# TengdaHan/TemporalAlignNet

Hardware: AMD Instinct MI355X
Metric: video-seq/sec (len=64, E6D6) at 1/2/4/8 MI355X; HTM-Align ROC-AUC parity (higher is better)
Workload: dtype bf16; 1 GPU; E6D6 len=64 bf16 stage-1 (init: multi-positive NCE only) train step (fwd+loss+bwd+AdamW), synthetic HTM-370K-shaped features, N~U[4,16] sentences/video; global_batch=128, per_gpu_batch=128, seq_len=64, parallelism=dp1

## Files before the change

### temporalalignnet_amd/csrc/tan_simnce.hip

```cpp
#include <type_traits>

#include "tan_mma.h"

namespace tal {

constexpr float S_TAU = 0.07f;
constexpr int S_TILE = 128 * 64 * 2;
constexpr int S_MAXCOLS = 2048;
constexpr int S_MAXCOLS_RES = 8192;

typedef const void __attribute__((address_space(1)))* sgptr_t;
typedef void __attribute__((address_space(3)))* slptr_t;

struct FamPtrs { void* p[8]; };
struct SimArgs {
    const bf16_t* V;
    const bf16_t* Tt;
    long t_stage_stride;
    const float* tgt;
    const unsigned char* col_invalid;
    const unsigned char* row_leak;
    float *rowsum, *possum_v;
    float *colpart, *pospart;
    const float *colsum, *possum_t;
// ... 11 lines not shown
    float* inv_v;
};

__device__ __forceinline__ void s_stage(const bf16_t* __restrict__ P, long ld, int outer0, int OUT, int k0, char* lds_tile,
                                        int wave, int lane) {
#pragma unroll
    for (int i = 0; i < 4; ++i) {
        const int piece = wave * 4 + i;
        const int row = piece * 8 + (lane >> 3), slot = lane & 7;
        const int chunk = slot ^ ((row >> 1) & 7);
        const int gr = min(outer0 + row, OUT - 1);
        __builtin_amdgcn_global_load_lds((sgptr_t)(P + (long)gr * ld + k0 + chunk * 8), (slptr_t)(lds_tile + piece * 1024), 16, 0, 0);
    }
}
__device__ __forceinline__ bf16x8 s_frag(const char* lds_tile, int o0, int ks, int lane) {
    const int row = o0 + (lane & 31), chunk = (ks >> 3) + (lane >> 5);
    return *reinterpret_cast<const bf16x8*>(lds_tile + row * 128 + (chunk ^ ((row >> 1) & 7)) * 16);
}

struct TileCtx {
    const unsigned char* col_invalid;
    const float* colsum; const float* g_t; bf16_t* dl;
    int R, Mp, s, m0, wm, wn, lane;
    float inv_tau;
    int cinv[2];
};

template <int MODE>
__device__ __forceinline__ void tile_done(const TileCtx& c, f32x16 (&acc)[2][2], float (&rowacc)[2][16], float* colacc, int ct) {
    const int c0 = ct * 128, R = c.R, Mp = c.Mp, lane = c.lane;
#pragma unroll
    for (int j = 0; j < 2; ++j) {
        const int col = c0 + c.wn * 64 + j * 32 + acc_col(lane);
        const bool col_ok = col < Mp;
        const bool col_valid = col_ok && !c.col_invalid[min(col, Mp - 1)];
        float csum = 0.f, bc = 0.f;
        if (MODE == 1) {
            const long idx = (long)c.s * Mp + min(col, Mp - 1);
            const float gt = c.g_t[idx], cs = c.colsum[idx];
            bc = col_ok ? gt / cs * c.inv_tau : 0.f;
        }
#pragma unroll
        for (int i = 0; i < 2; ++i)
#pragma unroll
            for (int r = 0; r < 16; ++r) {
                const int row = c.m0 + c.wm * 64 + i * 32 + acc_row(r, lane);
                float e = __expf((acc[i][j][r] - 1.0f) * c.inv_tau);
                if (!col_ok || row >= R) e = 0.f;
                if (MODE == 0) {
                    if (col_valid) rowacc[i][r] += e;
                    csum += e;
                } else {
                    const float g = e * ((col_valid ? rowacc[i][r] : 0.f) + bc);
                    if (col_ok && row < R) c.dl[((long)c.s * R + row) * Mp + col] = f2bf(g);
                }
            }
        if (MODE == 0 && col_ok) atomicAdd(&colacc[col], csum);
    }
}

template <int MODE>
__global__ __launch_bounds__(256, 2) void simnce_kernel(SimArgs a) {
    __shared__ __attribute__((aligned(1024))) char lds[4 * S_TILE + (MODE == 0 ? S_MAXCOLS * 4 : 0)];
    float* colacc = reinterpret_cast<float*>(lds + 4 * S_TILE);
    const int tid = threadIdx.x, lane = tid & 63;
    const int wave = __builtin_amdgcn_readfirstlane(tid >> 6);
    const int wm = wave >> 1, wn = wave & 1;
    const int npanel = gridDim.x;
    int wg = blockIdx.y * gridDim.x + blockIdx.x;
    {
        const int nwg = gridDim.x * gridDim.y, xcd = wg & 7, q = nwg >> 3, r = nwg & 7;
        wg = (xcd < r ? xcd * (q + 1) : r * (q + 1) + (xcd - r) * q) + (wg >> 3);
    }
    const int s = wg / npanel, panel = wg - s * npanel, m0 = panel * 128;
    const int R = a.R, Mp = a.Mp, Cw = a.C, nS = a.S;
    const bf16_t* V = a.V + (long)s * R * Cw;
    const bf16_t* Tt = a.Tt + (long)s * a.t_stage_stride;
    const int nk = Cw / 64, nct = (Mp + 127) / 128, nsteps = nct * nk;
    const float inv_tau = 1.0f / S_TAU;

    if (MODE == 0) {
        for (int c = tid; c < S_MAXCOLS; c += 256) colacc[c] = 0.f;
    }
    float rowacc[2][16];
#pragma unroll
    for (int i = 0; i < 2; ++i)
#pragma unroll
        for (int r = 0; r < 16; ++r) {
            rowacc[i][r] = 0.f;
            if (MODE == 1) {
                const int row = m0 + wm * 64 + i * 32 + acc_row(r, lane);
                const long idx = (long)s * R + min(row, R - 1);
                const float gv = a.g_v[idx], rs = a.rowsum[idx];
                rowacc[i][r] = row < R ? gv / rs * inv_tau : 0.f;
            }
        }
    TileCtx c;
    c.col_invalid = a.col_invalid; c.colsum = a.colsum; c.g_t = a.g_t; c.dl = a.dl;
    c.R = R; c.Mp = Mp; c.s = s; c.m0 = m0; c.wm = wm; c.wn = wn; c.lane = lane; c.inv_tau = inv_tau;

    f32x16 acc[2][2];
#define SIM_KSTEP(STEP, CUR, NXT)                                                                                          \
    {                                                                                                                      \
        const int step_ = (STEP);                                                                                          \
        const int ct_ = step_ / nk, kt_ = step_ - ct_ * nk;                                                                \
        if (step_ + 1 < nsteps) {                                                                                          \
            const int ct2 = (step_ + 1) / nk, kt2 = (step_ + 1) - ct2 * nk;                                                \
            s_stage(V, Cw, m0, R, kt2 * 64, lds + (NXT) * 2 * S_TILE, wave, lane);                                         \
            s_stage(Tt, Cw, ct2 * 128, Mp, kt2 * 64, lds + (NXT) * 2 * S_TILE + S_TILE, wave, lane);                       \
        }                                                                                                                  \
        if (kt_ == 0) {                                                                                                    \
            _Pragma("unroll") for (int i = 0; i < 2; ++i) _Pragma("unroll") for (int j = 0; j < 2; ++j) acc_zero(acc[i][j]); \
        }                                                                                                                  \
        _Pragma("unroll") for (int ks = 0; ks < 64; ks += 16) {                                                            \
            bf16x8 af[2], bfr[2];                                                                                          \
            _Pragma("unroll") for (int i = 0; i < 2; ++i) af[i] = s_frag(lds + (CUR) * 2 * S_TILE, wm * 64 + i * 32, ks, lane); \
            _Pragma("unroll") for (int j = 0; j < 2; ++j)                                                                  \
                bfr[j] = s_frag(lds + (CUR) * 2 * S_TILE + S_TILE, wn * 64 + j * 32, ks, lane);                            \
            _Pragma("unroll") for (int i = 0; i < 2; ++i) _Pragma("unroll") for (int j = 0; j < 2; ++j)                    \
                acc[i][j] = __builtin_amdgcn_mfma_f32_32x32x16_bf16(af[i], bfr[j], acc[i][j], 0, 0, 0);                    \
        }                                                                                                                  \
        if (kt_ == nk - 1) tile_done<MODE>(c, acc, rowacc, colacc, ct_);                                   \
        asm volatile("s_waitcnt vmcnt(0)" ::: "memory");                                                                   \
        __syncthreads();                                                                                                   \
    }

    s_stage(V, Cw, m0, R, 0, lds, wave, lane);
    s_stage(Tt, Cw, 0, Mp, 0, lds + S_TILE, wave, lane);
    asm volatile("s_waitcnt vmcnt(0)" ::: "memory");
    __syncthreads();
    for (int step = 0; step < nsteps; step += 2) {
        SIM_KSTEP(step, 0, 1)
        if (step + 1 < nsteps) SIM_KSTEP(step + 1, 1, 0)
    }
#undef SIM_KSTEP

    if (MODE == 0) {
#pragma unroll
        for (int i = 0; i < 2; ++i)
#pragma unroll
            for (int r = 0; r < 16; ++r) {
                float v = rowacc[i][r];
#pragma unroll
                for (int o = 16; o > 0; o >>= 1) v += __shfl_xor(v, o, 64);
                const int row = m0 + wm * 64 + i * 32 + acc_row(r, lane);
                if ((lane & 31) == 0 && row < R) unsafeAtomicAdd(a.rowsum + (long)s * R + row, v);
            }
        __syncthreads();
        float* cp = a.colpart + ((long)panel * nS + s) * Mp;
        for (int cc = tid; cc < Mp; cc += 256) cp[cc] = colacc[cc];
    }
}

template <int MODE>
__device__ __forceinline__ void tile_done_res(const TileCtx& c, f32x16 (&acc)[2][2], float (&rowacc)[2][16], float* colrow, int ct) {
    const int c0 = ct * 128, R = c.R, Mp = c.Mp, lane = c.lane;
#pragma unroll
    for (int j = 0; j < 2; ++j) {
        const int col = c0 + c.wn * 64 + j * 32 + acc_col(lane);
        const bool col_ok = col < Mp;
        const bool col_valid = col_ok && !(c.cinv[j] >= 0 ? c.cinv[j] : (int)c.col_invalid[min(col, Mp - 1)]);
        float csum = 0.f, bc = 0.f, e_prev = 0.f;
        unsigned pk[4] = {0u, 0u, 0u, 0u};
        const float k1 = 1.4426950408889634f * c.inv_tau, cmask = col_ok ? 1.0f : 0.0f, vmask = col_valid ? 1.0f : 0.0f;
        const bool rows_full = c.m0 + 128 <= R;
        if (MODE == 1) {
            const long idx = (long)c.s * Mp + min(col, Mp - 1);
            const float gt = c.g_t[idx], cs = c.colsum[idx];
            bc = col_ok ? gt / cs * c.inv_tau : 0.f;
        }
#pragma unroll
        for (int i = 0; i < 2; ++i)
#pragma unroll
            for (int r = 0; r < 16; ++r) {
                const int row = c.m0 + c.wm * 64 + i * 32 + acc_row(r, lane);
                float e = __builtin_amdgcn_exp2f(fmaf(acc[i][j][r], k1, -k1)) * cmask;
                if (!rows_full && row >= R) e = 0.f;
                if (MODE == 0) {
                    rowacc[i][r] = fmaf(e, vmask, rowacc[i][r]);
                    csum += e;
                    if (c.dl) {
                        if (r & 1) pk[(r >> 1) & 3] = f2bf2(e_prev, e);
                        e_prev = e;
                        if ((r & 7) == 7)
                            reinterpret_cast<uint4*>(c.dl)[((i * 2 + j) * 2 + (r >> 3)) * 64 + lane] = make_uint4(pk[0], pk[1], pk[2], pk[3]);
                    }
                } else {
                    const float g = e * ((col_valid ? rowacc[i][r] : 0.f) + bc);
                    if (col_ok && row < R) c.dl[((long)c.s * R + row) * Mp + col] = f2bf(g);
                }
            }
        if (MODE == 0) {
            csum += __shfl_xor(csum, 32, 64);
            if (lane < 32 && col_ok) colrow[col] = csum;
        }
    }
}

template <int J, int END, typename F>
__device__ __forceinline__ void pn_static_for_s(F&& f) {
    if constexpr (J < END) {
        f(std::integral_constant<int, J>{});
        pn_static_for_s<J + 1, END>(f);
    }
}

__global__ __launch_bounds__(256) void simnce_pack_text_kernel(const bf16_t* __restrict__ Tt, long t_stage_stride, char* __restrict__ Tp,
                                                               long tp_stage_stride, int Mp, float* __restrict__ zero, long nzero) {
    const int cb = blockIdx.x, st = blockIdx.y, lane = threadIdx.x & 63, w = threadIdx.x >> 6;
    if (zero)
        for (long i = ((long)blockIdx.y * gridDim.x + blockIdx.x) * 256 + threadIdx.x; i < nzero; i += (long)gridDim.x * gridDim.y * 256) zero[i] = 0.f;
    const bf16_t* src = Tt + (long)st * t_stage_stride + (long)min(cb * 32 + (lane & 31), Mp - 1) * 512 + 8 * (lane >> 5);
    char* dst = Tp + (long)st * tp_stage_stride + (long)cb * 32 * 1024 + lane * 16;
    uint4 v[8];
#pragma unroll
    for (int i = 0; i < 8; ++i) v[i] = *reinterpret_cast<const uint4*>(src + (w * 8 + i) * 16);
#pragma unroll
    for (int i = 0; i < 8; ++i) *reinterpret_cast<uint4*>(dst + (long)(w * 8 + i) * 1024) = v[i];
}

template <int MODE>
__global__ __launch_bounds__(512) void simnce_res_kernel(SimArgs a) {
    __shared__ __attribute__((aligned(1024))) char lds[8 * S_TILE];
    const int tid = threadIdx.x, lane = tid & 63;
    const int wave = __builtin_amdgcn_readfirstlane(tid >> 6);
    const int grp = wave >> 2, gw = wave & 3, wm = gw >> 1, wn = gw & 1;
    const int npanel = a.npanel;
    int wg = blockIdx.x, half = -1;
    if (wg < a.nfull) {
        const int nwg = a.nfull, xcd = wg & 7, q = nwg >> 3, r = nwg & 7;
        wg = (xcd < r ? xcd * (q + 1) : r * (q + 1) + (xcd - r) * q) + (wg >> 3);
    } else {
        half = (wg - a.nfull) & 1;
        wg = a.nfull + ((wg - a.nfull) >> 1);
    }
    const int s = wg / npanel, panel = wg - s * npanel, m0 = panel * 128;
    const int R = a.R, Mp = a.Mp, Cw = a.C, nS = a.S;
    const bf16_t* V = a.V + (long)s * R * Cw;
    const int nct = (Mp + 127) / 128;
    const float inv_tau = 1.0f / S_TAU;

    float rowacc[2][16];
#pragma unroll
    for (int i = 0; i < 2; ++i)
#pragma unroll
        for (int r = 0; r < 16; ++r) {
            rowacc[i][r] = 0.f;
            if (MODE == 1) {
                const int row = m0 + wm * 64 + i * 32 + acc_row(r, lane);
                const long idx = (long)s * R + min(row, R - 1);
                const float gv = a.g_v[idx], rs = a.rowsum[idx];
                rowacc[i][r] = row < R ? gv / rs * inv_tau : 0.f;
            }
        }
    TileCtx c;
    c.col_invalid = a.col_invalid; c.colsum = a.colsum; c.g_t = a.g_t; c.dl = a.dl;
    c.R = R; c.Mp = Mp; c.s = s; c.m0 = m0; c.wm = wm; c.wn = wn; c.lane = lane; c.inv_tau = inv_tau;
    float* colrow = MODE == 0 ? a.colpart + ((long)(2 * panel + wm) * nS + s) * Mp : nullptr;

    f32x16 acc[2][2];
    constexpr int RD = MODE == 0 ? 8 : 4;
    struct BF { bf16x8 f[2]; };
    BF ring[RD];
    const char* Tp = a.Tp + (long)s * a.tp_stage_stride;
    auto load_b = [&](BF& dst, int ct, int ks) __attribute__((always_inline)) {
        const char* pb = Tp + ((long)((ct * 4 + wn * 2) * 32 + ks)) * 1024 + lane * 16;
        dst.f[0] = *reinterpret_cast<const bf16x8*>(pb);
        dst.f[1] = *reinterpret_cast<const bf16x8*>(pb + 32 * 1024);
    };
    const int nall = (nct - grp + 1) / 2;
    const int kbase = half == 1 ? (nall + 1) / 2 : 0;
    const int ngrp = half < 0 ? nall : (half == 0 ? (nall + 1) / 2 : nall / 2);
    const int rot = ngrp > 0 ? (panel * 7 + s * 3) % ngrp : 0;
    if (ngrp > 0) {
        pn_static_for_s<0, RD>([&](auto jc) { constexpr int J = decltype(jc)::value; load_b(ring[J], 2 * (kbase + rot) + grp, J); });
    }
    if (MODE == 0 && a.inv_v) {
        const bf16_t* X = reinterpret_cast<const bf16_t*>(a.xraw.p[s]);
#pragma unroll
        for (int kt = 0; kt < 4; ++kt) {
            char* tile = lds + (grp * 4 + kt) * S_TILE;
#pragma unroll
            for (int i = 0; i < 4; ++i) {
                const int piece = gw * 4 + i;
                const int row = piece * 8 + (lane >> 3), slot = lane & 7;
                const int chunk = slot ^ ((row >> 1) & 7);
                const int gr = min(m0 + row, R - 1);
                const long sr = (long)(gr / a.T) * a.x_grp_rows + a.x_off + gr % a.T;
                __builtin_amdgcn_global_load_lds((sgptr_t)(X + sr * Cw + (grp * 4 + kt) * 64 + chunk * 8), (slptr_t)(tile + piece * 1024), 16, 0, 0);
            }
        }
        asm volatile("s_waitcnt vmcnt(0)" ::: "memory");
        __syncthreads();
        bf16_t* vout = const_cast<bf16_t*>(V);
#pragma unroll 1
        for (int i0 = 0; i0 < 16; i0 += 4) {
            uint4 raw[4];
            char* ap[4];
#pragma unroll
            for (int j = 0; j < 4; ++j) {
                const int row = wave * 16 + i0 + j;
                ap[j] = lds + (lane >> 3) * S_TILE + row * 128 + (((lane & 7) ^ ((row >> 1) & 7)) * 16);
                raw[j] = *reinterpret_cast<const uint4*>(ap[j]);
            }
#pragma unroll
            for (int j = 0; j < 4; ++j) {
                const int row = wave * 16 + i0 + j;
                const unsigned w[4] = {raw[j].x, raw[j].y, raw[j].z, raw[j].w};
                float x[8];
#pragma unroll
                for (int e = 0; e < 4; ++e) { x[2 * e] = __uint_as_float(w[e] << 16); x[2 * e + 1] = __uint_as_float(w[e] & 0xffff0000u); }
                float q = ((x[0] * x[0] + x[1] * x[1]) + (x[2] * x[2] + x[3] * x[3])) + ((x[4] * x[4] + x[5] * x[5]) + (x[6] * x[6] + x[7] * x[7]));
                const float inv = 1.0f / sqrtf(wave_sum(q));
                uint4 y;
                y.x = f2bf2(x[0] * inv, x[1] * inv); y.y = f2bf2(x[2] * inv, x[3] * inv);
                y.z = f2bf2(x[4] * inv, x[5] * inv); y.w = f2bf2(x[6] * inv, x[7] * inv);
                *reinterpret_cast<uint4*>(ap[j]) = y;
                if (m0 + row < R) {
                    *reinterpret_cast<uint4*>(vout + (long)(m0 + row) * Cw + lane * 8) = y;
                    if (lane == 0) a.inv_v[(long)s * R + m0 + row] = inv;
                }
            }
        }
    } else {
#pragma unroll
        for (int kt = 0; kt < 4; ++kt) s_stage(V, Cw, m0, R, (grp * 4 + kt) * 64, lds + (grp * 4 + kt) * S_TILE, gw, lane);
        asm volatile("s_waitcnt vmcnt(0)" ::: "memory");
    }
    __syncthreads();
    bf16x8 afA[2], afB[2];
#pragma unroll
    for (int i = 0; i < 2; ++i) afA[i] = s_frag(lds, wm * 64 + i * 32, 0, lane);
    for (int it = 0; it < ngrp; ++it) {
        const int k_ = it + rot < ngrp ? it + rot : it + rot - ngrp, kn_ = k_ + 1 < ngrp ? k_ + 1 : 0;
        const int ct_ = 2 * (kbase + k_) + grp, ctn_ = 2 * (kbase + kn_) + grp;
        const bool more = it + 1 < ngrp;
#pragma unroll
        for (int i = 0; i < 2; ++i)
#pragma unroll
            for (int j = 0; j < 2; ++j) acc_zero(acc[i][j]);
#pragma unroll
        for (int j = 0; j < 2; ++j) c.cinv[j] = a.col_invalid[min(ct_ * 128 + wn * 64 + j * 32 + (lane & 31), Mp - 1)];
        pn_static_for_s<0, 32>([&](auto jc) {
            constexpr int KS = decltype(jc)::value;
            BF& Bf = ring[KS % RD];
            bf16x8(&af)[2] = (KS & 1) ? afB : afA;
            bf16x8(&an)[2] = (KS & 1) ? afA : afB;
#ifndef TAN_SIM_LAB
#define TAN_SIM_LAB 0
#endif
            if constexpr (!(TAN_SIM_LAB & 2)) {
                constexpr int KN = (KS + 1) & 31;
                const char* vn_ = lds + (KN >> 2) * S_TILE;
#pragma unroll
                for (int i = 0; i < 2; ++i) an[i] = s_frag(vn_, wm * 64 + i * 32, (KN & 3) * 16, lane);
            } else {
#pragma unroll
                for (int i = 0; i < 2; ++i) asm volatile("" : "+v"(an[i]));
            }
#pragma unroll
            for (int i = 0; i < 2; ++i)
#pragma unroll
                for (int j = 0; j < 2; ++j) acc[i][j] = __builtin_amdgcn_mfma_f32_32x32x16_bf16(af[i], Bf.f[j], acc[i][j], 0, 0, 0);
            if constexpr (!(TAN_SIM_LAB & 1)) {
                if constexpr (KS + RD < 32) load_b(Bf, ct_, KS + RD);
                else if (more) load_b(Bf, ctn_, KS + RD - 32);
            } else {
                asm volatile("" : "+v"(Bf.f[0]), "+v"(Bf.f[1]));
            }
            __builtin_amdgcn_sched_barrier(0);
        });
        if (MODE == 0 && a.ekeep && !(TAN_SIM_LAB & 4)) c.dl = a.ekeep + ((((long)s * npanel + panel) * nct + ct_) * 4 + gw) * 4096;
        if constexpr (!(TAN_SIM_LAB & 8)) tile_done_res<MODE>(c, acc, rowacc, colrow, ct_);
        else {
#pragma unroll
            for (int i = 0; i < 2; ++i)
#pragma unroll
                for (int j = 0; j < 2; ++j) asm volatile("" : "+v"(acc[i][j]));
        }
    }

    if (MODE == 0) {
#pragma unroll
        for (int i = 0; i < 2; ++i)
#pragma unroll
            for (int r = 0; r < 16; ++r) {
                float v = rowacc[i][r];
#pragma unroll
                for (int o = 16; o > 0; o >>= 1) v += __shfl_xor(v, o, 64);
                const int row = m0 + wm * 64 + i * 32 + acc_row(r, lane);
                if ((lane & 31) == 0 && row < R) unsafeAtomicAdd(a.rowsum + (long)s * R + row, v);
            }
    }
    if (MODE == 1 && a.diag) {
        asm volatile("s_waitcnt vmcnt(0)" ::: "memory");
        __builtin_amdgcn_fence(__ATOMIC_RELEASE, "workgroup");
        __syncthreads();
        __builtin_amdgcn_fence(__ATOMIC_ACQUIRE, "workgroup");
        const int T = a.T, N = a.N;
        const int nrow = min(128, R - m0);
        for (int i = tid; i < nrow * N; i += 512) {
            const int lr = i / N, k = i - lr * N, row = m0 + lr;
            const int b = row / T, t = row - b * T;
            const int m = a.colmap ? a.colmap[b * N + k] : b * N + k;
            if (m < 0) continue;
            bf16_t* out = a.dl + ((long)s * R + row) * Mp + m;
            if (a.row_leak && a.row_leak[row]) { *out = 0; continue; }
            if (a.tgt[((long)b * T + t) * N + k] == 0.f) continue;
            const long ri = (long)s * R + row, ci = (long)s * Mp + m;
            const float e = __expf((a.diag[(((long)s * a.B + b) * T + t) * N + k] - 1.0f) * inv_tau);
            const float pv = a.possum_v[ri], pt = a.possum_t[ci];
            float corr = 0.f;
            if (!a.col_invalid[m] && pv > 0.f) corr += a.g_v[ri] / pv;
            if (pt > 0.f) corr += a.g_t[ci] / pt;
            *out = f2bf(bf2f(*out) - e * corr * inv_tau);
        }
    }
}

__global__ __launch_bounds__(256) void simnce_dl_kept_kernel(SimArgs a, int npanel, int nct) {
    constexpr int LD = 136;
    __shared__ __attribute__((aligned(16))) bf16_t tile[128 * LD];
    __shared__ float rf[128], cf[128];
    __shared__ unsigned char cv[128];
    __shared__ int crange[2];
    const int tid = threadIdx.x, s = blockIdx.y;
    const int panel = blockIdx.x / nct, ct = blockIdx.x - panel * nct;
    const int R = a.R, Mp = a.Mp, T = a.T, N = a.N, m0 = panel * 128, c0 = ct * 128;
    const float inv_tau = 1.0f / S_TAU;
    if (tid == 0) { crange[0] = 0x7fffffff; crange[1] = -1; }
    __syncthreads();
    if (a.diag) {
        const int b_lo = m0 / T, b_hi = min(m0 + 127, R - 1) / T;
        for (int p = b_lo * N + tid; p < (b_hi + 1) * N; p += 256) {
            const int m = a.colmap ? a.colmap[p] : p;
            if (m >= 0) { atomicMin(&crange[0], m); atomicMax(&crange[1], m); }
        }
    }
    if (tid < 128) {
        const long ri = (long)s * R + min(m0 + tid, R - 1);
        rf[tid] = a.g_v[ri] / a.rowsum[ri] * inv_tau;
    } else {
        const int c = tid - 128, col = min(c0 + c, Mp - 1);
        const long ci = (long)s * Mp + col;
        cf[c] = a.g_t[ci] / a.colsum[ci] * inv_tau;
        cv[c] = !a.col_invalid[col];
    }
    __syncthreads();
    const uint4* E = reinterpret_cast<const uint4*>(a.ekeep) + (((long)s * npanel + panel) * nct + ct) * 2048;
    uint4 ev[8];
#pragma unroll
    for (int n = 0; n < 8; ++n) ev[n] = E[tid + 256 * n];
#pragma unroll
    for (int n = 0; n < 8; ++n) {
        const int v = tid + 256 * n;
        const int gw = v >> 9, ij = (v >> 7) & 3, q = (v >> 6) & 1, ln = v & 63;
        const int col = (gw & 1) * 64 + (ij & 1) * 32 + (ln & 31);
        const unsigned w[4] = {ev[n].x, ev[n].y, ev[n].z, ev[n].w};
        const float c = cf[col];
        const bool ok = cv[col];
#pragma unroll
        for (int j = 0; j < 4; ++j) {
            const int row = (gw >> 1) * 64 + (ij >> 1) * 32 + acc_row(8 * q + 2 * j, ln);
            tile[row * LD + col] = f2bf(__uint_as_float(w[j] << 16) * ((ok ? rf[row] : 0.f) + c));
            tile[(row + 1) * LD + col] = f2bf(__uint_as_float(w[j] & 0xffff0000u) * ((ok ? rf[row + 1] : 0.f) + c));
        }
    }
    __syncthreads();
    if (a.diag && crange[0] <= c0 + 127 && crange[1] >= c0) {
        const int nrow = min(128, R - m0);
        for (int i = tid; i < nrow * N; i += 256) {
            const int lr = i / N, k = i - lr * N, row = m0 + lr;
            const int b = row / T, t = row - b * T;
            const int m = a.colmap ? a.colmap[b * N + k] : b * N + k;
            if (m < c0 || m >= c0 + 128 || m >= Mp) continue;
            bf16_t* out = tile + lr * LD + (m - c0);
            if (a.row_leak && a.row_leak[row]) { *out = 0; continue; }
            if (a.tgt[((long)b * T + t) * N + k] == 0.f) continue;
            const long ri = (long)s * R + row, ci = (long)s * Mp + m;
            const float e = __expf((a.diag[(((long)s * a.B + b) * T + t) * N + k] - 1.0f) * inv_tau);
            const float pv = a.possum_v[ri], pt = a.possum_t[ci];
            float corr = 0.f;
            if (!a.col_invalid[m] && pv > 0.f) corr += a.g_v[ri] / pv;
            if (pt > 0.f) corr += a.g_t[ci] / pt;
            *out = f2bf(bf2f(*out) - e * corr * inv_tau);
        }
        __syncthreads();
    }
    const bool vec = (Mp & 7) == 0;
    for (int q = tid; q < 128 * 16; q += 256) {
        const int lr = q >> 4, cc = (q & 15) * 8, row = m0 + lr, col = c0 + cc;
        if (row >= R || col >= Mp) continue;
        bf16_t* dst = a.dl + ((long)s * R + row) * Mp + col;
        if (vec) *reinterpret_cast<uint4*>(dst) = *reinterpret_cast<const uint4*>(tile + lr * LD + cc);
        else for (int j = 0; j < 8 && col + j < Mp; ++j) dst[j] = tile[lr * LD + cc + j];
    }
}

__global__ __launch_bounds__(256) void simnce_corr_kernel(const float* __restrict__ diag, const float* __restrict__ tgt,
                                                          const unsigned char* __restrict__ col_invalid, const unsigned char* __restrict__ row_leak,
                                                          const float* __restrict__ possum_v, const float* __restrict__ possum_t,
                                                          const float* __restrict__ g_v, const float* __restrict__ g_t, float* __restrict__ corr,
                                                          int B, int T, int N, const int* __restrict__ colmap, int Mp,
                                                          float* __restrict__ zero = nullptr, long nzero = 0) {
    const int b = blockIdx.x, s = blockIdx.y;
    const int R = B * T;
    const float inv_tau = 1.0f / S_TAU;
    const float* blk = diag + ((long)s * B + b) * T * N;
    const float* tg = tgt + (long)b * T * N;
    float* out = corr + ((long)s * B + b) * T * N;
    if (zero)
        for (long i = ((long)blockIdx.y * gridDim.x + blockIdx.x) * 256 + threadIdx.x; i < nzero; i += (long)gridDim.x * gridDim.y * 256) zero[i] = 0.f;
    constexpr int U = 4;
    for (int i0 = threadIdx.x; i0 < T * N; i0 += 256 * U) {
        int cc[U]; long r[U], c[U]; bool in[U], leak[U];
        float tgv[U], bl[U], pv[U], gv[U], pt[U], gt[U]; unsigned char inval[U];
#pragma unroll
        for (int j = 0; j < U; ++j) {
            const int i = min(i0 + j * 256, T * N - 1);
            const int t = i / N, k = i - t * N;
            const int m = colmap ? colmap[b * N + k] : b * N + k;
            in[j] = m >= 0 && m < Mp;
            cc[j] = min(max(m, 0), Mp - 1);
            r[j] = (long)s * R + b * T + t;
            c[j] = (long)s * Mp + cc[j];
            leak[j] = row_leak && row_leak[b * T + t];
            tgv[j] = tg[i]; bl[j] = blk[i]; inval[j] = col_invalid[cc[j]];
            pv[j] = possum_v[r[j]]; gv[j] = g_v[r[j]]; pt[j] = possum_t[c[j]]; gt[j] = g_t[c[j]];
        }
#pragma unroll
        for (int j = 0; j < U; ++j) {
            if (i0 + j * 256 >= T * N) continue;
            float v = 0.f;
            if (in[j]) {
                if (leak[j]) v = INFINITY;
                else if (tgv[j] != 0.f) {
                    const float e = __expf((bl[j] - 1.0f) * inv_tau);
                    float cr = 0.f;
                    if (!inval[j] && pv[j] > 0.f) cr += gv[j] / pv[j];
                    if (pt[j] > 0.f) cr += gt[j] / pt[j];
                    v = e * cr * inv_tau;
                }
            }
            out[i0 + j * 256] = v;
        }
    }
}
// ... 358 lines not shown
                              const unsigned char* __restrict__ col_invalid, int ncols, const float* __restrict__ colsum,
                              const float* __restrict__ possum_t, float* __restrict__ t_terms, long SM, float log_rows) {
    const float log_cols = (long)blockIdx.x * blockDim.x < SR ? block_log_count_zero(col_invalid, ncols) : 0.f;
    const long i = (long)blockIdx.x * blockDim.x + threadIdx.x;
    if (i >= SR + SM) return;
    const bool rows = i < SR;
    const long k = rows ? i : i - SR;
    const float all = rows ? rowsum[k] : colsum[k], pos = rows ? possum_v[k] : possum_t[k], lc = rows ? log_cols : log_rows;
    const float shift = 1.0f / S_TAU;
    const float den = logf(all) + shift;
    const float num = pos > 0.f ? logf(pos) + shift : -6e4f + lc;
    (rows ? v_terms : t_terms)[k] = den - num;
}

}

using namespace tal;

extern "C" int tan_simnce_max_cols(void) {
    SimArgs a{};
    a.C = 512;
    return res_enabled(a) ? S_MAXCOLS_RES : S_MAXCOLS;
}

static long simnce_corr_floats(int S, int B, int T, int N) { return (long)S * B * T * N + 128 * 32 + 8; }

extern "C" long tan_simnce_ws_floats(int S, int B, int T, int N) {
    const long R = (long)B * T, Mp = (long)B * N;
    return 2 * (long)cdiv(R, 128) * S * Mp + (long)S * B * T * N + (long)S * cdiv(Mp, 128) * 128 * 512 / 2 + 4 + simnce_corr_floats(S, B, T, N);
}
static float* simnce_corr_ptr(float* ws, int S, int B, int T, int N) {
    const long R = (long)B * T, Mp = (long)B * N;
    float* p = ws + 2 * (long)cdiv(R, 128) * S * Mp + (long)S * B * T * N + (long)S * cdiv(Mp, 128) * 128 * 512 / 2 + 4;
    return (float*)(((uintptr_t)p + 15) & ~(uintptr_t)15);
}
static int simnce_corr_launch(const SimArgs& a, const float* diag, float* corr, hipStream_t st) {
    hipLaunchKernelGGL(simnce_corr_kernel, dim3(a.B, a.S), dim3(256), 0, st, diag, a.tgt, a.col_invalid, a.row_leak, (const float*)a.possum_v,
                       a.possum_t, a.g_v, a.g_t, corr, a.B, a.T, a.N, a.colmap, a.Mp);
    hipError_t e = hipGetLastError();
    return e == hipSuccess ? 0 : (int)e;
}

static int simnce_common(SimArgs& a, int S, int B, int T, int N, int C) {
    a.S = S; a.B = B; a.T = T; a.N = N; a.C = C; a.R = B * T; a.Mp = B * N;
    if (S <= 0 || B <= 0 || T <= 0 || N <= 0 || C <= 0 || C % 64 != 0) return TAN_ERR_BAD_ARG;
    if (((uintptr_t)a.V % 16) || ((uintptr_t)a.Tt % 16)) return TAN_ERR_BAD_ARG;
    return 0;
}

__global__ __launch_bounds__(256) void simnce_blocks_kernel(const bf16_t* __restrict__ V, const bf16_t* __restrict__ tn_blocks,
                                                            long tb_stage_stride, float* __restrict__ diag, int B, int T, int N, long R) {
    constexpr int C = 512;
    const int b = blockIdx.x, s = blockIdx.y, lane = threadIdx.x & 63, wave = threadIdx.x >> 6;
    const int t0 = (blockIdx.z * 4 + wave) * 32;
    if (t0 >= T) return;
    const int hi8 = 8 * (lane >> 5);
    const bf16_t* arow = V + ((long)s * R + (long)b * T + min(t0 + (lane & 31), T - 1)) * C + hi8;
    float* out = diag + ((long)s * B + b) * T * N;
    for (int n0 = 0; n0 < N; n0 += 32) {
        const bf16_t* brow = tn_blocks + (long)s * tb_stage_stride + ((long)b * N + min(n0 + (lane & 31), N - 1)) * C + hi8;
        f32x16 acc;
        acc_zero(acc);
#pragma unroll 8
        for (int ks = 0; ks < C; ks += 16) {
            const bf16x8 fa = *reinterpret_cast<const bf16x8*>(arow + ks);
            const bf16x8 fb = *reinterpret_cast<const bf16x8*>(brow + ks);
            acc = __builtin_amdgcn_mfma_f32_32x32x16_bf16(fa, fb, acc, 0, 0, 0);
        }
        const int n = n0 + acc_col(lane);
#pragma unroll
        for (int r = 0; r < 16; ++r) {
            const int t = t0 + acc_row(r, lane);
            if (t < T && n < N) out[t * N + n] = acc[r];
        }
    }
}

static int simnce_diag_blocks(const SimArgs& a, const bf16_t* tn_blocks, long tb_stage_stride, float* diag, hipStream_t st) {
    if (a.C == 512 && (((uintptr_t)a.V | (uintptr_t)tn_blocks) % 16) == 0 && tb_stage_stride % 8 == 0) {
        hipLaunchKernelGGL(simnce_blocks_kernel, dim3(a.B, a.S, cdiv(a.T, 128)), dim3(256), 0, st, a.V, tn_blocks, tb_stage_stride, diag,
                           a.B, a.T, a.N, (long)a.R);
        hipError_t e = hipGetLastError();
        return e == hipSuccess ? 0 : (int)e;
    }
    const bool one_launch = tb_stage_stride == (long)a.B * a.N * a.C;
    for (int s = 0; s < (one_launch ? 1 : a.S); ++s) {
        tan_gemm_desc d{};
        d.dtype = TAN_BF16; d.out_dtype = TAN_F32;
        d.M = a.T; d.N = a.N; d.K = a.C; d.a_kc = 1; d.b_kc = 1;
        d.A = a.V + (long)s * a.R * a.C; d.lda = a.C;
        d.B = tn_blocks + (long)s * tb_stage_stride; d.ldb = a.C;
        d.C = diag + (long)s * a.B * a.T * a.N; d.ldc = a.N;
        d.split_k = 1; d.alpha = 1.0f;
        d.batch = one_launch ? a.S * a.B : a.B;
        d.sA = (long)a.T * a.C; d.sB = (long)a.N * a.C; d.sC = (long)a.T * a.N;
        int rc = tan_gemm(&d, st);
        if (rc) return rc;
    }
    return 0;
}

static int simnce_cus() {
    static const int n = [] { int dev = 0, v = 0; if (hipGetDevice(&dev) != hipSuccess || hipDeviceGetAttribute(&v, hipDeviceAttributeMultiprocessorCount, dev) != hipSuccess || v <= 0) v = 256; return v; }();
    return n;
}

static int simnce_pack_text(SimArgs& a, float* ws_after_diag, hipStream_t st, float* zero = nullptr, long nzero = 0) {
    char* base = (char*)(((uintptr_t)ws_after_diag + 15) & ~(uintptr_t)15);
    const int nblk = cdiv(a.Mp, 128) * 4;
    const bool shared = a.t_stage_stride == 0;
    a.Tp = base;
    a.tp_stage_stride = shared ? 0 : (long)nblk * 32 * 1024;
    hipLaunchKernelGGL(simnce_pack_text_kernel, dim3(nblk, shared ? 1 : a.S), dim3(256), 0, st, a.Tt, a.t_stage_stride, base, a.tp_stage_stride, a.Mp, zero, nzero);
    hipError_t e = hipGetLastError();
    return e == hipSuccess ? 0 : (int)e;
}

static int simnce_fwd_impl(const void* vn, const void* tn, long t_stage_stride, const float* tgt, const unsigned char* col_invalid,
                           const unsigned char* row_leak, float* rowsum, float* colsum, float* possum_v, float* possum_t,
                           float* v_terms, float* t_terms, float* ws, int S, int B, int T, int N, int C, const void* tn_blocks,
                           long tb_stage_stride, const int* colmap, int Mc, int phases, void* ekeep, void* stream) {
    TAN_REQUIRE(vn && tn && tgt && col_invalid && rowsum && colsum && possum_v && possum_t && v_terms && t_terms && ws);
    TAN_REQUIRE(!colmap || (tn_blocks && Mc > 0 && Mc <= B * N));
    if (phases == 0) phases = TAN_SIM_SWEEP | TAN_SIM_DIAG | TAN_SIM_TERMS;
    SimArgs a{};
    a.V = (const bf16_t*)vn; a.Tt = (const bf16_t*)tn; a.t_stage_stride = t_stage_stride;
    a.tgt = tgt; a.col_invalid = col_invalid; a.row_leak = row_leak;
    a.rowsum = rowsum; a.possum_v = possum_v;
    int rc = simnce_common(a, S, B, T, N, C);
    if (rc) return rc;
    const int npanel = cdiv(a.R, 128);
    a.colpart = ws;
    float* diag = ws + 2 * (long)npanel * S * a.Mp;
    if (colmap) a.Mp = Mc;
    else { tn_blocks = tn; tb_stage_stride = t_stage_stride; }
    if (a.Mp > (res_enabled(a) ? S_MAXCOLS_RES : S_MAXCOLS)) return TAN_ERR_BAD_ARG;
    hipStream_t st = (hipStream_t)stream;
    const long SM = (long)S * a.Mp, SR = (long)S * a.R;
    if (phases & TAN_SIM_SWEEP) {
        const bool res = res_enabled(a);
        const bool zero_rows = !(phases & TAN_SIM_ACC_ROWS);
        if (zero_rows && !res) {
            hipError_t e = hipMemsetAsync(rowsum, 0, sizeof(float) * (size_t)S * a.R, st);
            if (e != hipSuccess) return (int)e;
        }
        const int prec = prof_begin(st, TAN_PROF_SIMNCE, 2.0 * S * a.R * (double)a.Mp * C);
        if (ekeep && !res) return TAN_ERR_BAD_ARG;
        a.ekeep = (bf16_t*)ekeep;
        if (res && (rc = simnce_pack_text(a, diag + (long)S * B * T * N, st, zero_rows ? rowsum : nullptr, (long)S * a.R))) return rc;
        if (res) {
            const int items = npanel * S, ncu = simnce_cus(), rem = items % ncu;
            a.npanel = npanel;
            a.nfull = items; (void)ncu; (void)rem;
            hipLaunchKernelGGL((simnce_res_kernel<0>), dim3(a.nfull + 2 * (items - a.nfull)), dim3(512), 0, st, a);
        }
        else hipLaunchKernelGGL((simnce_kernel<0>), dim3(npanel, S), dim3(256), 0, st, a);
        prof_end(st, prec);
        TAN_LAUNCH_CHECK();
        hipLaunchKernelGGL(simnce_col_finalize, dim3(cdiv(SM, 64)), dim3(64), 0, st, a.colpart, colsum, res ? 2 * npanel : npanel, SM);
    }
    if (phases & TAN_SIM_DIAG) {
        if ((rc = simnce_diag_blocks(a, (const bf16_t*)tn_blocks, tb_stage_stride, diag, st))) return rc;
        hipLaunchKernelGGL((simnce_diag_kernel<false>), dim3(B, S), dim3(256), sizeof(float) * 2 * (size_t)(T + N), st, diag, tgt, col_invalid, row_leak, rowsum, colsum,
                           possum_v, possum_t, (const float*)nullptr, (const float*)nullptr, (bf16_t*)nullptr, B, T, N, colmap, a.Mp);
    }
    if (phases & TAN_SIM_TERMS) {
        hipLaunchKernelGGL(simnce_terms2, dim3(cdiv(SR + SM, 256)), dim3(256), 0, st, rowsum, possum_v, v_terms, SR, a.col_invalid, a.Mp, colsum,
                           possum_t, t_terms, SM, logf((float)a.R));
    }
    TAN_LAUNCH_CHECK();
    return 0;
}

extern "C" int tan_simnce_fwd(const void* vn, const void* tn, long t_stage_stride, const float* tgt, const unsigned char* col_invalid,
                              const unsigned char* row_leak, float* rowsum, float* colsum, float* possum_v, float* possum_t,
                              float* v_terms, float* t_terms, float* ws, int S, int B, int T, int N, int C, const void* tn_blocks,
                              long tb_stage_stride, const int* colmap, int Mc, int phases, void* stream) {
    return simnce_fwd_impl(vn, tn, t_stage_stride, tgt, col_invalid, row_leak, rowsum, colsum, possum_v, possum_t, v_terms, t_terms, ws,
                           S, B, T, N, C, tn_blocks, tb_stage_stride, colmap, Mc, phases, nullptr, stream);
}

extern "C" int tan_simnce_keeps(int C) {
    SimArgs a{}; a.C = C;
    return res_enabled(a) ? 1 : 0;
}

extern "C" long tan_simnce_keep_elems(int S, int R, int Mp) { return (long)S * cdiv(R, 128) * cdiv(Mp, 128) * 16384; }

extern "C" int tan_simnce_fwd_keep(const void* vn, const void* tn, long t_stage_stride, const float* tgt, const unsigned char* col_invalid,
                                   const unsigned char* row_leak, float* rowsum, float* colsum, float* possum_v, float* possum_t,
                                   float* v_terms, float* t_terms, float* ws, int S, int B, int T, int N, int C, const void* tn_blocks,
                                   long tb_stage_stride, const int* colmap, int Mc, int phases, void* e_keep, void* stream) {
    TAN_REQUIRE(e_keep);
    return simnce_fwd_impl(vn, tn, t_stage_stride, tgt, col_invalid, row_leak, rowsum, colsum, possum_v, possum_t, v_terms, t_terms, ws,
                           S, B, T, N, C, tn_blocks, tb_stage_stride, colmap, Mc, phases, e_keep, stream);
}

static int simnce_bwd_impl(const void* vn, const void* tn, long t_stage_stride, const float* tgt,
                           const unsigned char* col_invalid, const unsigned char* row_leak, const float* rowsum,
                           const float* colsum, const float* possum_v, const float* possum_t, const float* g_v, const float* g_t,
                           void* dl, float* ws, int S, int B, int T, int N, int C, const void* tn_blocks, long tb_stage_stride,
                           const int* colmap, int Mc, int phases, const void* ekeep, void* dvn, void* stream) {
    TAN_REQUIRE(vn && tn && tgt && col_invalid && rowsum && colsum && possum_v && possum_t && g_v && g_t && (dl || dvn) && ws);
    TAN_REQUIRE(!colmap || (tn_blocks && Mc > 0 && Mc <= B * N));
    if (phases == 0) phases = TAN_SIM_SWEEP | TAN_SIM_DIAG;
    TAN_REQUIRE(!dvn || (ekeep && (phases & TAN_SIM_SWEEP) && (uintptr_t)dvn % 16 == 0));
    SimArgs a{};
    a.V = (const bf16_t*)vn; a.Tt = (const bf16_t*)tn; a.t_stage_stride = t_stage_stride;
    a.tgt = tgt; a.col_invalid = col_invalid; a.row_leak = row_leak;
    a.rowsum = (float*)rowsum; a.possum_v = (float*)possum_v; a.colsum = colsum; a.possum_t = possum_t;
    a.g_v = g_v; a.g_t = g_t; a.dl = (bf16_t*)dl;
    int rc = simnce_common(a, S, B, T, N, C);
    if (rc) return rc;
    hipStream_t st = (hipStream_t)stream;
    float* diag = ws + 2 * (long)cdiv(a.R, 128) * S * a.Mp;
    if (colmap) a.Mp = Mc;
    else { tn_blocks = tn; tb_stage_stride = t_stage_stride; }
    if (a.Mp > (res_enabled(a) ? S_MAXCOLS_RES : S_MAXCOLS)) return TAN_ERR_BAD_ARG;
    if (ekeep && (phases & TAN_SIM_SWEEP)) {
        const bool tail = (phases & TAN_SIM_DIAG) != 0;
        if (tail && !(phases & TAN_SIM_DIAG_KEEP) && (rc = simnce_diag_blocks(a, (const bf16_t*)tn_blocks, tb_stage_stride, diag, st))) return rc;
        a.ekeep = (bf16_t*)ekeep; a.diag = tail ? diag : nullptr; a.colmap = colmap;
        if (dvn && tail) {
            float* corr = simnce_corr_ptr(ws, S, B, T, N);
            if (!(phases & TAN_SIM_CORR_KEEP) && (rc = simnce_corr_launch(a, diag, corr, st))) return rc;
            a.corr = corr;
        }
        if (dvn && (a.Mp % 8 || N > DV_MAX_N || a.Mp > 32767)) return TAN_ERR_BAD_ARG;
        if (dvn) {
            const int npanel = cdiv(a.R, 128), nct = cdiv(a.Mp, 128);
            char* TpT = (char*)(((uintptr_t)(diag + (long)S * B * T * N) + 15) & ~(uintptr_t)15);
            const bool shared = a.t_stage_stride == 0;
            const long tpt_stride = shared ? 0 : (long)nct * 128 * 1024;
            hipLaunchKernelGGL(simnce_pack_textT_kernel, dim3(nct * 4, shared ? 1 : S), dim3(256), 0, st, a.Tt, a.t_stage_stride, TpT, tpt_stride, a.Mp);
            TAN_LAUNCH_CHECK();
            static std::atomic<unsigned long long> lds_done{0};
        const hipError_t attr = ensure_dyn_lds((const void*)simnce_dl_dvn_kernel, DV_LDS_B, lds_done);
            if (attr != hipSuccess) return (int)attr;
            const int prec = prof_begin(st, TAN_PROF_GEMM_BF16 + 1, 2.0 * S * a.R * (double)a.Mp * C);
            hipLaunchKernelGGL(simnce_dl_dvn_kernel, dim3(npanel * S), dim3(512), DV_LDS_B, st, a, npanel, nct, (const char*)TpT, tpt_stride, (bf16_t*)dvn, FamL2{});
            prof_end(st, prec);
            TAN_LAUNCH_CHECK();
            return 0;
        }
        hipLaunchKernelGGL(simnce_dl_kept_kernel, dim3(cdiv(a.R, 128) * cdiv(a.Mp, 128), S), dim3(256), 0, st, a, cdiv(a.R, 128), cdiv(a.Mp, 128));
        TAN_LAUNCH_CHECK();
        return 0;
    }
    if (phases & TAN_SIM_SWEEP) {
        const bool res = res_enabled(a);
        const bool tail = res && (phases & TAN_SIM_DIAG);
        if (tail && !(phases & TAN_SIM_DIAG_KEEP) && (rc = simnce_diag_blocks(a, (const bf16_t*)tn_blocks, tb_stage_stride, diag, st))) return rc;
        const int prec = prof_begin(st, TAN_PROF_SIMNCE, 2.0 * S * a.R * (double)a.Mp * C);
        if (res) {
            a.diag = tail ? diag : nullptr; a.colmap = colmap;
            if ((rc = simnce_pack_text(a, diag + (long)S * B * T * N, st))) return rc;
            a.npanel = cdiv(a.R, 128); a.nfull = a.npanel * S;
            hipLaunchKernelGGL((simnce_res_kernel<1>), dim3(a.nfull), dim3(512), 0, st, a);
            if (tail) phases &= ~TAN_SIM_DIAG;
        } else hipLaunchKernelGGL((simnce_kernel<1>), dim3(cdiv(a.R, 128), S), dim3(256), 0, st, a);
        prof_end(st, prec);
        TAN_LAUNCH_CHECK();
    }
    if (phases & TAN_SIM_DIAG) {
        if (!(phases & TAN_SIM_DIAG_KEEP) && (rc = simnce_diag_blocks(a, (const bf16_t*)tn_blocks, tb_stage_stride, diag, st))) return rc;
        hipLaunchKernelGGL((simnce_diag_kernel<true>), dim3(B, S), dim3(256), 0, st, diag, tgt, col_invalid, row_leak, (float*)rowsum,
                           (float*)colsum, (float*)possum_v, (float*)possum_t, g_v, g_t, (bf16_t*)dl, B, T, N, colmap, a.Mp);
    }
    TAN_LAUNCH_CHECK();
    return 0;
}

extern "C" int tan_simnce_bwd_dl(const void* vn, const void* tn, long t_stage_stride, const float* tgt,
                                 const unsigned char* col_invalid, const unsigned char* row_leak, const float* rowsum,
                                 const float* colsum, const float* possum_v, const float* possum_t, const float* g_v, const float* g_t,
                                 void* dl, float* ws, int S, int B, int T, int N, int C, const void* tn_blocks, long tb_stage_stride,
                                 const int* colmap, int Mc, int phases, void* stream) {
    return simnce_bwd_impl(vn, tn, t_stage_stride, tgt, col_invalid, row_leak, rowsum, colsum, possum_v, possum_t, g_v, g_t, dl, ws,
                           S, B, T, N, C, tn_blocks, tb_stage_stride, colmap, Mc, phases, nullptr, nullptr, stream);
}

extern "C" int tan_simnce_bwd_dl_kept(const void* e_keep, const void* vn, const void* tn, long t_stage_stride, const float* tgt,
                                      const unsigned char* col_invalid, const unsigned char* row_leak, const float* rowsum,
                                      const float* colsum, const float* possum_v, const float* possum_t, const float* g_v,
                                      const float* g_t, void* dl, float* ws, int S, int B, int T, int N, int C, const void* tn_blocks,
                                      long tb_stage_stride, const int* colmap, int Mc, int phases, void* stream) {
    TAN_REQUIRE(e_keep);
    return simnce_bwd_impl(vn, tn, t_stage_stride, tgt, col_invalid, row_leak, rowsum, colsum, possum_v, possum_t, g_v, g_t, dl, ws,
                           S, B, T, N, C, tn_blocks, tb_stage_stride, colmap, Mc, phases, e_keep, nullptr, stream);
}

extern "C" int tan_simnce_bwd_dl_dvn_kept(const void* e_keep, const void* vn, const void* tn, long t_stage_stride, const float* tgt,
                                          const unsigned char* col_invalid, const unsigned char* row_leak, const float* rowsum,
                                          const float* colsum, const float* possum_v, const float* possum_t, const float* g_v,
                                          const float* g_t, void* dl, void* d_vn, float* ws, int S, int B, int T, int N, int C,
                                          const void* tn_blocks, long tb_stage_stride, const int* colmap, int Mc, int phases, void* stream) {
    TAN_REQUIRE(e_keep && d_vn && C == 512);
    if (phases == 0) phases = TAN_SIM_SWEEP | TAN_SIM_DIAG;
    return simnce_bwd_impl(vn, tn, t_stage_stride, tgt, col_invalid, row_leak, rowsum, colsum, possum_v, possum_t, g_v, g_t, dl, ws,
                           S, B, T, N, C, tn_blocks, tb_stage_stride, colmap, Mc, phases, e_keep, d_vn, stream);
}

namespace tal {

struct FamText {
    FamPtrs xs;
    long grp_rows, off;
// ... 433 lines not shown
```

Measured before the change: 31450 video-seq/s.

## Restructure resident simNCE kernel: split stats/dl epilogues, new LDS panel layout

Splits the tile epilogue into a stats path (row/col exp sums, optional bf16 keep) and a gradient path. The stats path masks out-of-range rows once per tile by setting accumulators to -inf and folds column validity into the exp bias. A no-keep variant (MODE 2) is added and dispatched when ekeep is null. The LDS tile layout is reorganised into 64-row panels and staged directly with global_load_lds, with a simplified fragment address computation. The outer loop is kept rolled, and the final B prefetch now wraps to the first column tile instead of being guarded, which issues a few redundant loads on the last iteration.

```diff
diff --git a/temporalalignnet_amd/csrc/tan_simnce.hip b/temporalalignnet_amd/csrc/tan_simnce.hip
--- a/temporalalignnet_amd/csrc/tan_simnce.hip
+++ b/temporalalignnet_amd/csrc/tan_simnce.hip
@@ -187,23 +187,60 @@
     }
 }
 
-template <int MODE>
-__device__ __forceinline__ void tile_done_res(const TileCtx& c, f32x16 (&acc)[2][2], float (&rowacc)[2][16], float* colrow, int ct) {
+template <bool KEEP>
+__device__ __forceinline__ void tile_stats_res(const TileCtx& c, f32x16 (&acc)[2][2], float (&rowacc)[2][16], float* colrow, int ct, bool full) {
+    const int c0 = ct * 128, Mp = c.Mp, lane = c.lane;
+    const float k1 = 1.4426950408889634f * c.inv_tau;
+    if (!full) {
+        int left = c.R - (c.m0 + c.wm * 64 + 4 * (lane >> 5));
+        asm volatile("" : "+v"(left));
+#pragma unroll
+        for (int i = 0; i < 2; ++i)
+#pragma unroll
+            for (int r = 0; r < 16; ++r)
+                if (i * 32 + acc_row(r, 0) >= left) {
+#pragma unroll
+                    for (int j = 0; j < 2; ++j) acc[i][j][r] = -INFINITY;
+                }
+    }
+#pragma unroll
+    for (int j = 0; j < 2; ++j) {
+        const int col = c0 + c.wn * 64 + j * 32 + acc_col(lane);
+        const bool col_ok = col < Mp;
+        const float bias = col_ok ? -k1 : -INFINITY, vmask = col_ok && !c.cinv[j] ? 1.0f : 0.0f;
+        float csum = 0.f, e_prev = 0.f;
+        unsigned pk[4] = {0u, 0u, 0u, 0u};
+#pragma unroll
+        for (int i = 0; i < 2; ++i)
+#pragma unroll
+            for (int r = 0; r < 16; ++r) {
+                float e = __builtin_amdgcn_exp2f(fmaf(acc[i][j][r], k1, bias));
+                rowacc[i][r] = fmaf(e, vmask, rowacc[i][r]);
+                csum += e;
+                if (KEEP) {
+                    if (r & 1) pk[(r >> 1) & 3] = f2bf2(e_prev, e);
+                    e_prev = e;
+                    if ((r & 7) == 7)
+                        reinterpret_cast<uint4*>(c.dl)[((i * 2 + j) * 2 + (r >> 3)) * 64 + lane] = make_uint4(pk[0], pk[1], pk[2], pk[3]);
+                }
+            }
+        csum += __shfl_xor(csum, 32, 64);
+        if (lane < 32 && col_ok) colrow[col] = csum;
+    }
+}
+
+__device__ __forceinline__ void tile_dl_res(const TileCtx& c, f32x16 (&acc)[2][2], float (&rowacc)[2][16], int ct) {
     const int c0 = ct * 128, R = c.R, Mp = c.Mp, lane = c.lane;
 #pragma unroll
     for (int j = 0; j < 2; ++j) {
         const int col = c0 + c.wn * 64 + j * 32 + acc_col(lane);
         const bool col_ok = col < Mp;
         const bool col_valid = col_ok && !(c.cinv[j] >= 0 ? c.cinv[j] : (int)c.col_invalid[min(col, Mp - 1)]);
-        float csum = 0.f, bc = 0.f, e_prev = 0.f;
-        unsigned pk[4] = {0u, 0u, 0u, 0u};
-        const float k1 = 1.4426950408889634f * c.inv_tau, cmask = col_ok ? 1.0f : 0.0f, vmask = col_valid ? 1.0f : 0.0f;
+        const float k1 = 1.4426950408889634f * c.inv_tau, cmask = col_ok ? 1.0f : 0.0f;
         const bool rows_full = c.m0 + 128 <= R;
-        if (MODE == 1) {
-            const long idx = (long)c.s * Mp + min(col, Mp - 1);
-            const float gt = c.g_t[idx], cs = c.colsum[idx];
-            bc = col_ok ? gt / cs * c.inv_tau : 0.f;
-        }
+        const long idx = (long)c.s * Mp + min(col, Mp - 1);
+        const float gt = c.g_t[idx], cs = c.colsum[idx];
+        const float bc = col_ok ? gt / cs * c.inv_tau : 0.f;
 #pragma unroll
         for (int i = 0; i < 2; ++i)
 #pragma unroll
@@ -211,24 +248,9 @@
                 const int row = c.m0 + c.wm * 64 + i * 32 + acc_row(r, lane);
                 float e = __builtin_amdgcn_exp2f(fmaf(acc[i][j][r], k1, -k1)) * cmask;
                 if (!rows_full && row >= R) e = 0.f;
-                if (MODE == 0) {
-                    rowacc[i][r] = fmaf(e, vmask, rowacc[i][r]);
-                    csum += e;
-                    if (c.dl) {
-                        if (r & 1) pk[(r >> 1) & 3] = f2bf2(e_prev, e);
-                        e_prev = e;
-                        if ((r & 7) == 7)
-                            reinterpret_cast<uint4*>(c.dl)[((i * 2 + j) * 2 + (r >> 3)) * 64 + lane] = make_uint4(pk[0], pk[1], pk[2], pk[3]);
-                    }
-                } else {
-                    const float g = e * ((col_valid ? rowacc[i][r] : 0.f) + bc);
-                    if (col_ok && row < R) c.dl[((long)c.s * R + row) * Mp + col] = f2bf(g);
-                }
-            }
-        if (MODE == 0) {
-            csum += __shfl_xor(csum, 32, 64);
-            if (lane < 32 && col_ok) colrow[col] = csum;
-        }
+                const float g = e * ((col_valid ? rowacc[i][r] : 0.f) + bc);
+                if (col_ok && row < R) c.dl[((long)c.s * R + row) * Mp + col] = f2bf(g);
+            }
     }
 }
 
@@ -256,7 +278,9 @@
 
 template <int MODE>
 __global__ __launch_bounds__(512) void simnce_res_kernel(SimArgs a) {
+    constexpr bool STATS = MODE != 1;
     __shared__ __attribute__((aligned(1024))) char lds[8 * S_TILE];
+    auto panel_off = [](int kt, int row) __attribute__((always_inline)) { return ((row >> 6) << 16) + kt * (S_TILE / 2) + (row & 63) * 128; };
     const int tid = threadIdx.x, lane = tid & 63;
     const int wave = __builtin_amdgcn_readfirstlane(tid >> 6);
     const int grp = wave >> 2, gw = wave & 3, wm = gw >> 1, wn = gw & 1;
@@ -281,7 +305,7 @@
 #pragma unroll
         for (int r = 0; r < 16; ++r) {
             rowacc[i][r] = 0.f;
-            if (MODE == 1) {
+            if (!STATS) {
                 const int row = m0 + wm * 64 + i * 32 + acc_row(r, lane);
                 const long idx = (long)s * R + min(row, R - 1);
                 const float gv = a.g_v[idx], rs = a.rowsum[idx];
@@ -291,17 +315,18 @@
     TileCtx c;
     c.col_invalid = a.col_invalid; c.colsum = a.colsum; c.g_t = a.g_t; c.dl = a.dl;
     c.R = R; c.Mp = Mp; c.s = s; c.m0 = m0; c.wm = wm; c.wn = wn; c.lane = lane; c.inv_tau = inv_tau;
-    float* colrow = MODE == 0 ? a.colpart + ((long)(2 * panel + wm) * nS + s) * Mp : nullptr;
+    float* colrow = STATS ? a.colpart + ((long)(2 * panel + wm) * nS + s) * Mp : nullptr;
 
     f32x16 acc[2][2];
-    constexpr int RD = MODE == 0 ? 8 : 4;
+    constexpr int RD = STATS ? 8 : 4;
     struct BF { bf16x8 f[2]; };
     BF ring[RD];
     const char* Tp = a.Tp + (long)s * a.tp_stage_stride;
+    const unsigned lane16 = (unsigned)lane * 16u;
     auto load_b = [&](BF& dst, int ct, int ks) __attribute__((always_inline)) {
-        const char* pb = Tp + ((long)((ct * 4 + wn * 2) * 32 + ks)) * 1024 + lane * 16;
-        dst.f[0] = *reinterpret_cast<const bf16x8*>(pb);
-        dst.f[1] = *reinterpret_cast<const bf16x8*>(pb + 32 * 1024);
+        const char* pb = Tp + ((long)((ct * 4 + wn * 2) * 32 + ks)) * 1024;
+        dst.f[0] = *reinterpret_cast<const bf16x8*>(pb + lane16);
+        dst.f[1] = *reinterpret_cast<const bf16x8*>(pb + 32 * 1024 + lane16);
     };
     const int nall = (nct - grp + 1) / 2;
     const int kbase = half == 1 ? (nall + 1) / 2 : 0;
@@ -310,11 +335,10 @@
     if (ngrp > 0) {
         pn_static_for_s<0, RD>([&](auto jc) { constexpr int J = decltype(jc)::value; load_b(ring[J], 2 * (kbase + rot) + grp, J); });
     }
-    if (MODE == 0 && a.inv_v) {
+    if (STATS && a.inv_v) {
         const bf16_t* X = reinterpret_cast<const bf16_t*>(a.xraw.p[s]);
 #pragma unroll
         for (int kt = 0; kt < 4; ++kt) {
-            char* tile = lds + (grp * 4 + kt) * S_TILE;
 #pragma unroll
             for (int i = 0; i < 4; ++i) {
                 const int piece = gw * 4 + i;
@@ -322,7 +346,8 @@
                 const int chunk = slot ^ ((row >> 1) & 7);
                 const int gr = min(m0 + row, R - 1);
                 const long sr = (long)(gr / a.T) * a.x_grp_rows + a.x_off + gr % a.T;
-                __builtin_amdgcn_global_load_lds((sgptr_t)(X + sr * Cw + (grp * 4 + kt) * 64 + chunk * 8), (slptr_t)(tile + piece * 1024), 16, 0, 0);
+                __builtin_amdgcn_global_load_lds((sgptr_t)(X + sr * Cw + (grp * 4 + kt) * 64 + chunk * 8),
+                                                 (slptr_t)(lds + panel_off(grp * 4 + kt, piece * 8)), 16, 0, 0);
             }
         }
         asm volatile("s_waitcnt vmcnt(0)" ::: "memory");
@@ -335,7 +360,7 @@
 #pragma unroll
             for (int j = 0; j < 4; ++j) {
                 const int row = wave * 16 + i0 + j;
-                ap[j] = lds + (lane >> 3) * S_TILE + row * 128 + (((lane & 7) ^ ((row >> 1) & 7)) * 16);
+                ap[j] = lds + panel_off(lane >> 3, row) + (((lane & 7) ^ ((row >> 1) & 7)) * 16);
                 raw[j] = *reinterpret_cast<const uint4*>(ap[j]);
             }
 #pragma unroll
@@ -359,63 +384,83 @@
         }
     } else {
 #pragma unroll
-        for (int kt = 0; kt < 4; ++kt) s_stage(V, Cw, m0, R, (grp * 4 + kt) * 64, lds + (grp * 4 + kt) * S_TILE, gw, lane);
+        for (int kt = 0; kt < 4; ++kt)
+#pragma unroll
+            for (int i = 0; i < 4; ++i) {
+                const int piece = gw * 4 + i;
+                const int row = piece * 8 + (lane >> 3), chunk = (lane & 7) ^ ((row >> 1) & 7);
+                __builtin_amdgcn_global_load_lds((sgptr_t)(V + (long)min(m0 + row, R - 1) * Cw + (grp * 4 + kt) * 64 + chunk * 8),
+                                                 (slptr_t)(lds + panel_off(grp * 4 + kt, piece * 8)), 16, 0, 0);
+            }
         asm volatile("s_waitcnt vmcnt(0)" ::: "memory");
     }
     __syncthreads();
-    bf16x8 afA[2], afB[2];
-#pragma unroll
-    for (int i = 0; i < 2; ++i) afA[i] = s_frag(lds, wm * 64 + i * 32, 0, lane);
-    for (int it = 0; it < ngrp; ++it) {
-        const int k_ = it + rot < ngrp ? it + rot : it + rot - ngrp, kn_ = k_ + 1 < ngrp ? k_ + 1 : 0;
-        const int ct_ = 2 * (kbase + k_) + grp, ctn_ = 2 * (kbase + kn_) + grp;
-        const bool more = it + 1 < ngrp;
-#pragma unroll
-        for (int i = 0; i < 2; ++i)
-#pragma unroll
-            for (int j = 0; j < 2; ++j) acc_zero(acc[i][j]);
-#pragma unroll
-        for (int j = 0; j < 2; ++j) c.cinv[j] = a.col_invalid[min(ct_ * 128 + wn * 64 + j * 32 + (lane & 31), Mp - 1)];
-        pn_static_for_s<0, 32>([&](auto jc) {
-            constexpr int KS = decltype(jc)::value;
-            BF& Bf = ring[KS % RD];
-            bf16x8(&af)[2] = (KS & 1) ? afB : afA;
-            bf16x8(&an)[2] = (KS & 1) ? afA : afB;
 #ifndef TAN_SIM_LAB
 #define TAN_SIM_LAB 0
 #endif
-            if constexpr (!(TAN_SIM_LAB & 2)) {
-                constexpr int KN = (KS + 1) & 31;
-                const char* vn_ = lds + (KN >> 2) * S_TILE;
-#pragma unroll
-                for (int i = 0; i < 2; ++i) an[i] = s_frag(vn_, wm * 64 + i * 32, (KN & 3) * 16, lane);
+    const char* fbase = lds + (wm << 16) + (lane & 31) * 128;
+    const int fsw = (lane >> 5) ^ ((lane >> 1) & 7);
+    auto frag = [&](int kn, int i) __attribute__((always_inline)) {
+        return *reinterpret_cast<const bf16x8*>(fbase + (kn >> 2) * (S_TILE / 2) + i * 4096 + ((fsw ^ (2 * (kn & 3))) * 16));
+    };
+    const bool full = m0 + 128 <= R;
+    constexpr bool KEEP = MODE == 0 && !(TAN_SIM_LAB & 4);
+    {
+        bf16x8 afA[2], afB[2];
+#pragma unroll
+        for (int i = 0; i < 2; ++i) afA[i] = frag(0, i);
+#pragma unroll 1
+        for (int it = 0; it < ngrp; ++it) {
+            const int k_ = it + rot < ngrp ? it + rot : it + rot - ngrp, kn_ = k_ + 1 < ngrp ? k_ + 1 : 0;
+            const int ct_ = 2 * (kbase + k_) + grp, ctn_ = 2 * (kbase + kn_) + grp;
+#pragma unroll
+            for (int i = 0; i < 2; ++i)
+#pragma unroll
+                for (int j = 0; j < 2; ++j) acc_zero(acc[i][j]);
+#pragma unroll
+            for (int j = 0; j < 2; ++j) c.cinv[j] = a.col_invalid[min(ct_ * 128 + wn * 64 + j * 32 + (lane & 31), Mp - 1)];
+            pn_static_for_s<0, 32>([&](auto jc) {
+                constexpr int KS = decltype(jc)::value;
+                BF& Bf = ring[KS % RD];
+                bf16x8(&af)[2] = (KS & 1) ? afB : afA;
+                bf16x8(&an)[2] = (KS & 1) ? afA : afB;
+                if constexpr (!(TAN_SIM_LAB & 2)) {
+#pragma unroll
+                    for (int i = 0; i < 2; ++i) an[i] = frag((KS + 1) & 31, i);
+                } else {
+#pragma unroll
+                    for (int i = 0; i < 2; ++i) asm volatile("" : "+v"(an[i]));
+                }
+#pragma unroll
+                for (int i = 0; i < 2; ++i)
+#pragma unroll
+                    for (int j = 0; j < 2; ++j) {
+                        if constexpr (!(TAN_SIM_LAB & 16)) acc[i][j] = __builtin_amdgcn_mfma_f32_32x32x16_bf16(af[i], Bf.f[j], acc[i][j], 0, 0, 0);
+                        else asm volatile("" : "+v"(acc[i][j]) : "v"(af[i]), "v"(Bf.f[j]));
+                    }
+                if constexpr (!(TAN_SIM_LAB & 1)) {
+                    if constexpr (KS + RD < 32) load_b(Bf, ct_, KS + RD);
+                    else load_b(Bf, ctn_, KS + RD - 32);
+                } else {
+                    asm volatile("" : "+v"(Bf.f[0]), "+v"(Bf.f[1]));
+                }
+                __builtin_amdgcn_sched_barrier(0);
+            });
+            if constexpr (TAN_SIM_LAB & 8) {
+#pragma unroll
+                for (int i = 0; i < 2; ++i)
+#pragma unroll
+                    for (int j = 0; j < 2; ++j) asm volatile("" : "+v"(acc[i][j]));
+            } else if constexpr (STATS) {
+                if (KEEP) c.dl = a.ekeep + ((((long)s * npanel + panel) * nct + ct_) * 4 + gw) * 4096;
+                tile_stats_res<KEEP>(c, acc, rowacc, colrow, ct_, full);
             } else {
-#pragma unroll
-                for (int i = 0; i < 2; ++i) asm volatile("" : "+v"(an[i]));
-            }
-#pragma unroll
-            for (int i = 0; i < 2; ++i)
-#pragma unroll
-                for (int j = 0; j < 2; ++j) acc[i][j] = __builtin_amdgcn_mfma_f32_32x32x16_bf16(af[i], Bf.f[j], acc[i][j], 0, 0, 0);
-            if constexpr (!(TAN_SIM_LAB & 1)) {
-                if constexpr (KS + RD < 32) load_b(Bf, ct_, KS + RD);
-                else if (more) load_b(Bf, ctn_, KS + RD - 32);
-            } else {
-                asm volatile("" : "+v"(Bf.f[0]), "+v"(Bf.f[1]));
-            }
-            __builtin_amdgcn_sched_barrier(0);
-        });
-        if (MODE == 0 && a.ekeep && !(TAN_SIM_LAB & 4)) c.dl = a.ekeep + ((((long)s * npanel + panel) * nct + ct_) * 4 + gw) * 4096;
-        if constexpr (!(TAN_SIM_LAB & 8)) tile_done_res<MODE>(c, acc, rowacc, colrow, ct_);
-        else {
-#pragma unroll
-            for (int i = 0; i < 2; ++i)
-#pragma unroll
-                for (int j = 0; j < 2; ++j) asm volatile("" : "+v"(acc[i][j]));
-        }
-    }
-
-    if (MODE == 0) {
+                tile_dl_res(c, acc, rowacc, ct_);
+            }
+        }
+    }
+
+    if (STATS) {
 #pragma unroll
         for (int i = 0; i < 2; ++i)
 #pragma unroll
@@ -427,7 +472,7 @@
                 if ((lane & 31) == 0 && row < R) unsafeAtomicAdd(a.rowsum + (long)s * R + row, v);
             }
     }
-    if (MODE == 1 && a.diag) {
+    if (!STATS && a.diag) {
         asm volatile("s_waitcnt vmcnt(0)" ::: "memory");
         __builtin_amdgcn_fence(__ATOMIC_RELEASE, "workgroup");
         __syncthreads();
@@ -1092,7 +1137,8 @@
             const int items = npanel * S, ncu = simnce_cus(), rem = items % ncu;
             a.npanel = npanel;
             a.nfull = items; (void)ncu; (void)rem;
-            hipLaunchKernelGGL((simnce_res_kernel<0>), dim3(a.nfull + 2 * (items - a.nfull)), dim3(512), 0, st, a);
+            if (a.ekeep) hipLaunchKernelGGL((simnce_res_kernel<0>), dim3(a.nfull + 2 * (items - a.nfull)), dim3(512), 0, st, a);
+            else hipLaunchKernelGGL((simnce_res_kernel<2>), dim3(a.nfull + 2 * (items - a.nfull)), dim3(512), 0, st, a);
         }
         else hipLaunchKernelGGL((simnce_kernel<0>), dim3(npanel, S), dim3(256), 0, st, a);
         prof_end(st, prec);
```

Measured after the change: 31670 video-seq/s (median of 6 runs). No clear change (+0.7%).
